# granne/granne

Hardware: AMD Instinct MI355X
Metric: queries/sec (recall@10 alongside), 10M x 100-d angular, batch=1024 (higher is better)
Workload: dtype f32; 1 GPU; C2 (BASELINE.json configs[1]): 10000000 x 100-d f32 angular, i.i.d. uniform components, batch=1024, ef_search=50, k=10; n_elements=10000000, dim=100, batch=1024, ef_search=50, k=10

## Files before the change

granne_amd/_lib.py:

```python
import ctypes as C
import os

from . import build as _build

F32, I8, F16 = 0, 1, 2
UNUSED = 0xFFFFFFFF
BUILD_ALL = 0xFFFFFFFFFFFFFFFF

OK = 0
ERR_INVALID, ERR_HIP, ERR_NO_DEVICE, ERR_OVERFLOW, ERR_IO = -1, -2, -3, -4, -5

OPT_VISITED_SLOTS, OPT_FORCE_SLOW, OPT_SLOW_SLOTS, OPT_SLOW_BLOCKS, OPT_OVERFLOW_SLOTS = 1, 2, 3, 4, 5
OPT_VISITED16, OPT_VISITED16_LG, OPT_LAST_WALKER, OPT_SEARCH_DEPTH, OPT_INLINE_TAILS, OPT_SEEN_MIN = 6, 7, 8, 9, 10, 11
OPT_SKETCH = 12
OPT_COALESCE, OPT_COALESCE_MAX, OPT_COALESCE_WAIT_US, OPT_COALESCED_LAUNCHES, OPT_COALESCED_QUERIES = 13, 14, 15, 16, 17
OPT_LAST_COMPACT_ROWS = 18
OPT_LAST_SPLIT_TAIL = 19
OPT_LAST_SCAN = 20
(SCAN_NONE, SCAN_RING, SCAN_I8, SCAN_I8_CHUNKED, SCAN_B16_7_4, SCAN_B16_13_2, SCAN_B16_16_1, SCAN_B16_CHUNKED, SCAN_F32_52_4,
 SCAN_F32_100_2, SCAN_F32_128_1) = range(11)
EXACT_TOPK_KMAX = 1024
EXACT_TOPK_CAP = 4096
COALESCE_CALL_MAX = 64
COALESCE_MAX = 1024
# ... 42 lines not shown
    "granne_hip_device_count": (i32, [C.POINTER(i32)]),
    "granne_hip_index_create": (i32, [C.POINTER(vp), vp, u64, u32, i32, u32, vp, vp, vp, i32]),
    "granne_hip_index_create_csr": (i32, [C.POINTER(vp), vp, u64, u32, i32, u32, vp, vp, vp, i32]),
    "granne_hip_index_create_device": (i32, [C.POINTER(vp), vp, u64, u32, i32, u32, vp, vp, vp, i32, vp]),
    "granne_hip_index_destroy": (None, [vp]),
    "granne_hip_index_len": (u64, [vp]),
    "granne_hip_index_num_layers": (u32, [vp]),
    "granne_hip_index_layer_len": (u64, [vp, u32]),
    "granne_hip_index_dim": (u32, [vp]),
    "granne_hip_index_dtype": (i32, [vp]),
    "granne_hip_index_device": (i32, [vp]),
    "granne_hip_index_hbm_bytes": (u64, [vp]),
    "granne_hip_index_get_neighbors": (i32, [vp, u64, u32, vp, u32, C.POINTER(u32)]),
    "granne_hip_index_get_element": (i32, [vp, u64, vp]),
    "granne_hip_index_get_sketch": (i32, [vp, u64, u64, vp]),
    "granne_hip_search_batch": (i32, [vp, vp, u32, u32, u32, vp, vp, vp, vp]),
    "granne_hip_search_batch_device": (i32, [vp, vp, u32, u32, u32, vp, vp, vp, vp, vp, vp]),
    "granne_hip_search_batches_device": (i32, [vp, u32, vp, u32, u32, u32, vp, vp, vp, vp, vp, vp]),
    "granne_hip_search_begin_device": (i32, [vp, vp, u32, u32, u32, vp, vp, vp, vp, vp, vp, C.POINTER(u64)]),
    "granne_hip_search_end_device": (i32, [vp, u64, vp]),
    "granne_hip_device_malloc": (i32, [C.POINTER(vp), u64, i32]),
    "granne_hip_device_free": (i32, [vp, i32]),
    "granne_hip_copy_to_device": (i32, [vp, vp, u64, i32, vp]),
    "granne_hip_copy_to_host": (i32, [vp, vp, u64, i32, vp]),
    "granne_hip_stream_create": (i32, [C.POINTER(vp), i32]),
    "granne_hip_stream_destroy": (i32, [vp, i32]),
    "granne_hip_stream_synchronize": (i32, [vp, i32]),
    "granne_hip_event_create": (i32, [vp]),
    "granne_hip_event_destroy": (None, [vp]),
    "granne_hip_event_elapsed_ms": (i32, [vp, vp, vp]),
# ... 134 lines not shown
```

granne_amd/csrc/granne_hip.hip:

```cpp
#include <hip/hip_runtime.h>

#include <atomic>
#include <chrono>
#include <cstdarg>
#include <cstdio>
#include <cstdlib>
#include <cstring>
#include <memory>
#include <mutex>
#include <string>
#include <type_traits>
#include <vector>

#include "../../include/granne_hip.h"
#include "search_kernel.h"
#include "walk_fast.h"
#include "slow_kernel.h"
#include "util_kernels.h"
#include "brute_force.h"
#include "exact_topk.h"
#include "combiner.h"
#include "dev_mem.h"

using namespace granne_hip;
// ... 337 lines not shown
    const uint64_t n = ix->n_elements;
    const size_t bytes = (size_t)n * SKETCH_LINE;
    if (!ix->d_sketch) {
        size_t free_b = 0, total_b = 0;
        if (hipMemGetInfo(&free_b, &total_b) != hipSuccess) {
            (void)hipGetLastError();
            return GRANNE_HIP_OK;
        }
        if ((uint64_t)free_b < (uint64_t)bytes + total_b / 32u) return GRANNE_HIP_OK;
        if (ix->d_sketch.alloc(bytes) != hipSuccess) {
            (void)hipGetLastError();
            return GRANNE_HIP_OK;
        }
        ix->hbm_bytes += bytes;
    }
    hipLaunchKernelGGL(row_sketch_kernel, dim3(grid_for(n, 256)), dim3(256), 0, s, ix->d_elements.as<uint8_t>(), n, ix->row_stride, ix->dim,
                       ix->d_sketch.as<uint8_t>());
    HIP_TRY(hipGetLastError());
    return GRANNE_HIP_OK;
}

static int finish_layers(granne_hip_index* ix, hipStream_t s) {
    std::vector<LayerDev> h(ix->layers.size());
    ix->max_dev_width = 32;
    {
        int r = make_inline_tails(ix, s);
        if (r == 0) r = make_scan_norms(ix, s);
        if (r == 0) r = make_row_sketch(ix, s);
        if (r) return r;
    }
    DevBuf found_buf;
    std::vector<uint32_t> found(h.size(), 0u);
// ... 216 lines not shown
}

extern "C" int granne_hip_index_get_element(const granne_hip_index* ix, uint64_t idx, void* out) {
    if (!ix || !out) return fail(GRANNE_HIP_ERR_INVALID, "null argument");
    if (idx >= ix->n_elements) return fail(GRANNE_HIP_ERR_INVALID, "element index out of range");
    if (ix->se) return se_rows_to_host(*ix->se, idx, 1, 1, (float*)out);
    DeviceGuard g(ix->device);
    HIP_TRY(hipMemcpy(out, ix->d_elements.as<uint8_t>() + idx * ix->row_stride, (size_t)ix->dim * elem_size(ix->dtype),
                      hipMemcpyDeviceToHost));
    return GRANNE_HIP_OK;
}

extern "C" int granne_hip_index_get_sketch(const granne_hip_index* ix, uint64_t first, uint64_t count, void* out) {
    if (!ix || (!out && count)) return fail(GRANNE_HIP_ERR_INVALID, "null argument");
    GRANNE_HIP_COMPACT_UNSUPPORTED(ix, "get_sketch");
    if (!ix->d_sketch) return fail(GRANNE_HIP_ERR_INVALID, "the index holds no row sketches");
    if (first > ix->n_elements || count > ix->n_elements - first) return fail(GRANNE_HIP_ERR_INVALID, "rows out of range");
    if (count == 0) return GRANNE_HIP_OK;
    DeviceGuard g(ix->device);
    HIP_TRY(hipMemcpy(out, ix->d_sketch.as<uint8_t>() + first * SKETCH_LINE, (size_t)count * SKETCH_LINE, hipMemcpyDeviceToHost));
    return GRANNE_HIP_OK;
}

extern "C" int granne_hip_index_set_option(granne_hip_index* ix, int option, uint64_t value) {
    if (!ix) return fail(GRANNE_HIP_ERR_INVALID, "index is null");
    switch (option) {
    case GRANNE_HIP_OPT_VISITED_SLOTS:
        {
            const uint64_t odd = value ? value >> __builtin_ctzll(value) : 1;
            if (value != 0 && (value < 256 || value > 32768 || (odd != 1 && odd != 3)))
// ... 364 lines not shown
    else
        P.S = ef_walk <= 64 ? 1u : ef_walk <= 128 ? 2u : 4u;

    const int vmode = T.opt_visited16 ? (int)T.opt_visited16 : knobs().visited;
    const bool none = vmode == 4 || vmode == 0;
    const bool longest = walk_list_is_long((int)P.S, wide) || wide;
    uint32_t walk_lds;
    if (fast && !trail && ((none && !T.opt_visited_slots) || longest)) {
        const uint32_t touch_max = knobs().touch_max >= 0 ? (uint32_t)knobs().touch_max : 256u;
        const bool touch_shape = P.S == 1 && !wide && !streamed && !(i8 && T.stage_row_bytes != 128);
        P.v16 = (touch_shape && nq <= touch_max) ? 4 : 3;
        const uint64_t seen_min = knobs().seen_min >= 0 ? (uint64_t)knobs().seen_min : T.opt_seen_min;
        if (P.S <= 4 && !wide && !i8 && nq >= seen_min) P.v16 = 5;
        P.cr = P.v16 == 5 && !i8 && sketch_dim_ok(T.dim) && T.d_sketch != nullptr && knobs().compact_rows != 0;
        P.split = P.cr && !wide;
        walk_lds = fast_lds_bytes(i8, streamed, T.dim, T.stage_row_bytes, P.S, 0u, P.v16 == 5, wide);
        const uint32_t least = lds_query_bytes(T.stage_row_bytes) + 64u * 8u;
        if (walk_lds < least) walk_lds = least;
    } else {
        uint32_t want = T.opt_visited_slots ? (uint32_t)T.opt_visited_slots : next_pow2(ef_walk * 64u);
        if (!T.opt_visited_slots) {
            if (want < 1024) want = 1024;
            uint32_t cap = nq >= 4096 ? 4096u : 8192u;
            if (fast && P.S >= 8) cap = 4096u;
            if (want > cap) want = cap;
        }
        P.visited_slots = want;
        P.upper_slots = want < 1024 ? want : 1024;
        if (fast) {
            walk_lds = fast_lds_bytes(i8, streamed, T.dim, T.stage_row_bytes, P.S, P.visited_slots, false, wide);
        } else {
// ... 1282 lines not shown
```

granne_amd/csrc/search_kernel.h:

```cpp
#pragma once

#include "dist.h"
#include "wave_prims.h"
#include "sum_embeddings.h"
#include "f16.h"

namespace granne_hip {

constexpr int DT_F32 = 0;
constexpr int DT_I8 = 1;

struct LayerDev {
    const uint32_t* adj;
    uint64_t len;
    uint32_t width;
    uint32_t flags;
    const uint8_t* adjx;
    uint32_t adjx_stride;
    uint32_t reserved;
};
constexpr uint32_t LAYER_TWIN_ROWS = 1u;

constexpr uint32_t SKETCH_LINE = 128u;
constexpr uint32_t SKETCH_META = 112u;
constexpr uint32_t SKETCH_MAX_DIM = 112u;
__host__ __device__ constexpr bool sketch_dim_ok(uint32_t dim) { return dim == 100u; }

constexpr uint32_t MAX_LAUNCH_BATCHES = 32;
struct BatchIO {
    const uint8_t* queries;
    uint64_t* out_ids;
    float* out_dists;
    uint32_t* out_counts;
    uint64_t* out_stats;
};

struct SearchParams {
    const uint8_t* elements;
    uint64_t n_elements;
    uint32_t dim;
    uint32_t row_bytes;
// ... 548 lines not shown
```

granne_amd/csrc/util_kernels.h:

```cpp
#pragma once

#include "dist.h"
#include "ordered_sum.h"
#include "search_kernel.h"

namespace granne_hip {

__device__ __forceinline__ float sketch_ceil_sqrt(double S) {
    const double T = S * (1.0 + 0x1p-40);
    if (!(T <= (double)3.4028234663852886e38 * (double)3.4028234663852886e38)) return __builtin_inff();
    float f = (float)__builtin_sqrt(T);
    while ((double)f * (double)f < T) f = __uint_as_float(__float_as_uint(f) + 1u);
    while (f > 0.0f) {
        const float g = __uint_as_float(__float_as_uint(f) - 1u);
        if ((double)g * (double)g < T) break;
        f = g;
    }
    return f;
}

__global__ void row_sketch_kernel(const uint8_t* __restrict__ elements, uint64_t n, uint32_t row_stride, uint32_t dim,
                                  uint8_t* __restrict__ out) {
    for (uint64_t row = (uint64_t)blockIdx.x * blockDim.x + threadIdx.x; row < n; row += (uint64_t)gridDim.x * blockDim.x) {
        const float* x = reinterpret_cast<const float*>(elements + row * row_stride);
        uint32_t* o = reinterpret_cast<uint32_t*>(out + row * SKETCH_LINE);
        float m = 0.0f;
        bool finite = true;
        for (uint32_t i = 0; i < dim; ++i) {
            const float a = __builtin_fabsf(x[i]);
            finite = finite && a <= 3.4028234663852886e38f;
            m = a > m ? a : m;
        }
        const float s = finite ? (float)((double)m / 127.0) : 0.0f;
        double se = 0.0, sc = 0.0, sx = 0.0;
        for (uint32_t j = 0; j < SKETCH_META / 4u; ++j) {
            uint32_t w = 0;
            for (uint32_t t = 0; t < 4u; ++t) {
                const uint32_t i = j * 4u + t;
                if (i >= dim) break;
                const double xd = (double)x[i];
                double c = 0.0;
                if (s > 0.0f) {
                    c = __builtin_rint(xd / (double)s);
                    c = c < -127.0 ? -127.0 : (c > 127.0 ? 127.0 : c);
                }
                const double pc = (double)s * c, e = xd - pc;
                se = se + e * e;
                sc = sc + pc * pc;
                sx = sx + xd * xd;
                w |= ((uint32_t)(int32_t)c & 0xFFu) << (8u * t);
            }
            o[j] = w;
        }
        const float inf = __builtin_inff();
        o[SKETCH_META / 4u + 0u] = __float_as_uint(s);
        o[SKETCH_META / 4u + 1u] = __float_as_uint(finite ? sketch_ceil_sqrt(se) : inf);
        o[SKETCH_META / 4u + 2u] = __float_as_uint(finite ? sketch_ceil_sqrt(sc) : inf);
        o[SKETCH_META / 4u + 3u] = __float_as_uint(finite ? sketch_ceil_sqrt(sx) : inf);
    }
}

__global__ void relayout_rows_kernel(const uint8_t* __restrict__ src, uint8_t* __restrict__ dst, uint64_t n,
                                     uint32_t src_bytes, uint32_t dst_bytes) {
    const uint32_t units = dst_bytes >> 4;
    uint64_t total = n * units;
    for (uint64_t t = (uint64_t)blockIdx.x * blockDim.x + threadIdx.x; t < total;
         t += (uint64_t)gridDim.x * blockDim.x) {
        uint64_t row = t / units;
        uint32_t u = (uint32_t)(t - row * units);
        const uint8_t* s = src + row * src_bytes + (uint64_t)u * 16;
        uint32_t avail = (u * 16 < src_bytes) ? min(16u, src_bytes - u * 16) : 0u;
        uint32_t w[4] = {0, 0, 0, 0};
        uint8_t* wb = reinterpret_cast<uint8_t*>(w);
// ... 363 lines not shown
```

granne_amd/csrc/walk_fast.h:

```cpp
#pragma once

#include <type_traits>

#include "slow_kernel.h"

namespace granne_hip {

#ifndef GRANNE_HIP_PHASE_TIMERS
#define GRANNE_HIP_PHASE_TIMERS 0
#endif
#if GRANNE_HIP_PHASE_TIMERS
constexpr uint32_t PHASE_SLOTS = 48, PHASE_QUERIES = 4096;
__device__ uint64_t g_phase[PHASE_QUERIES * PHASE_SLOTS];
#define PT_MARK(i)                                                                   \
    do {                                                                             \
        asm volatile("" ::: "memory");                                               \
        __builtin_amdgcn_sched_barrier(0);                                           \
        const uint64_t now_ = __builtin_amdgcn_s_memtime();                          \
        const uint64_t dt_ = now_ - pt_last;                                         \
        if (pt_bottom) pt_b[i] += dt_; else pt_u[i] += dt_;                          \
        pt_last = now_;                                                              \
        __builtin_amdgcn_sched_barrier(0);                                           \
        asm volatile("" ::: "memory");                                               \
    } while (0)
// ... 182 lines not shown
    uint8_t* lds_q;
    uint64_t* mslot;
    uint32_t* vis_tab;
    uint32_t* vcache;
    float qh[QREG ? NB * 16 : 1];
    float qt[(QREG && TU) ? TU * 4 : 1];
    uint4 qi8[F32 ? 1 : 4 * NBI];
    float sy;
    uint32_t g_nbk, g_ngroups, g_tu;
    static constexpr bool NOVIS = V16 >= 3;
    static constexpr bool TOUCH = V16 == 4;
    static constexpr bool SEEN = V16 == 5;
    static_assert(!WIDE || V16 == 3, "layers of 64 ids: walked without a visited set only");
    static constexpr bool SK = SEEN && XT && sketch_dim_ok((uint32_t)DIM);
    static_assert(CR == 0 || (SK && (CR == 8 || CR == 4) && S <= 4), "the compacted row stage: the sketched launches, 8 or 4 lanes per row");
    int8_t* sk_qc;
    float sk_s, sk_r, sk_n;
    bool sk_on;
    static_assert(V16 == 0 || V16 == 3 || V16 == 4 || V16 == 5, "the exact 32-bit table, or no visited set (4: + rows touched ahead, 5: + revisits skipped before their rows are fetched)");
    typename std::conditional<V16 == 0, VisitedSet, VisitedNone>::type vis;
    List L;
    WalkStats st;
    bool bail;
    uint32_t theta;
#if GRANNE_HIP_PHASE_TIMERS
    uint64_t pt_b[16] = {}, pt_u[16] = {}, pt_last = 0, pt_t0 = 0;
    uint32_t pt_nb = 0, pt_nu = 0, pt_cnt[8] = {0, 0, 0, 0, 0, 0, 0, 0};
    bool pt_bottom = false;
#endif

    __device__ __forceinline__ FastWalker(const SearchParams& p_, uint8_t* smem) : p(p_) {
        lane = threadIdx.x;
        h = lane & 1u;
        R = lane >> 1;
        const uint32_t qb = fast_query_bytes(!F32, GEN, p.dim, p.row_bytes, (uint32_t)S, V16 == 5);
        g_nbk = p.dim / 32u;
        g_ngroups = (g_nbk + GEN_GROUP - 1u) / GEN_GROUP;
        g_tu = ((p.dim & 31u) + 3u) / 4u;
        lds_q = smem;
        mslot = reinterpret_cast<uint64_t*>(smem + qb);
        fimg = reinterpret_cast<uint64_t*>(smem + qb + List::IMAGE_KEYS * 8u);
        vcache = reinterpret_cast<uint32_t*>(smem + qb + List::IMAGE_KEYS * 8u + (LONG_LIST ? FIMG_KEYS * 8u : 0u));
        fkey = KEY_INF;
        nF = nM = 0;
        m_un = 0;
        m_un_key = KEY_INF;
        lost_bits = 0xFFFFFFFFu;
        vis_tab = reinterpret_cast<uint32_t*>(smem + qb + List::IMAGE_KEYS * 8u + (LONG_LIST ? FIMG_KEYS * 8u : 0u) + VSLOTS * 4u);
        st.n_dist = st.n_expand = st.n_adj = 0;
        bail = false;
        sy = 0.0f;
        sk_qc = reinterpret_cast<int8_t*>(vis_tab);
        sk_s = sk_r = sk_n = 0.0f;
        sk_on = false;
        vis.init_walker();
    }

    __device__ __forceinline__ void load_query(uint32_t qi) {
        if constexpr (F32) {
            const float* q = reinterpret_cast<const float*>(query_io(p, qi).q);
            if constexpr (QREG) {
#pragma unroll
                for (int b = 0; b < NB; ++b)
// ... 44 lines not shown
            m = t > m ? t : m;
        }
        const float s = m / 127.0f;
        const float inv = m > 0.0f ? 127.0f / m : 0.0f;
        float c0 = __builtin_rintf(v0 * inv), c1 = __builtin_rintf(v1 * inv);
        c0 = c0 < -127.0f ? -127.0f : (c0 > 127.0f ? 127.0f : c0);
        c1 = c1 < -127.0f ? -127.0f : (c1 > 127.0f ? 127.0f : c1);
        const float e0 = __builtin_fmaf(-s, c0, v0), e1 = __builtin_fmaf(-s, c1, v1);
        float ee = __builtin_fmaf(e1, e1, e0 * e0), nn = __builtin_fmaf(v1, v1, v0 * v0);
        for (int o = 32; o > 0; o >>= 1) {
            ee += __shfl_xor(ee, o, 64);
            nn += __shfl_xor(nn, o, 64);
        }
        sk_qc[lane] = (int8_t)(int)c0;
        sk_qc[lane + 64u] = (int8_t)(int)c1;
        asm volatile("" ::: "memory");
        sk_s = __int_as_float(__builtin_amdgcn_readfirstlane(__float_as_int(s)));
        sk_r = __int_as_float(__builtin_amdgcn_readfirstlane(__float_as_int(__builtin_sqrtf(ee) * (1.0f + 0x1p-8f) + 0x1p-58f)));
        sk_n = __int_as_float(__builtin_amdgcn_readfirstlane(__float_as_int(__builtin_sqrtf(nn) * (1.0f + 0x1p-8f) + 0x1p-58f)));
        sk_on = fin;
    }

    struct RowRegs {
        float4 v[NB ? NB : 1][4];
        float4 vt[GEN ? 8 : (TU ? TU : 1)];
        uint4 x[4 * NBI];
        const uint8_t* row;
    };

    __device__ __forceinline__ void load_group(RowRegs& rr, uint32_t g) {
// ... 47 lines not shown
            const uint8_t* line = p.sketch + (size_t)nb * SKETCH_LINE + h * 64u;
#pragma unroll
            for (int k = 0; k < 4; ++k) rr.v[0][k] = *reinterpret_cast<const float4*>(line + k * 16);
        }
        asm volatile("" ::: "memory");
        int ip = 0;
#pragma unroll
        for (int k = 0; k < 4; ++k) {
            const uint4 qq = *reinterpret_cast<const uint4*>(sk_qc + h * 64u + k * 16);
            ip = dot4_i8(__float_as_uint(rr.v[0][k].x), qq.x, ip);
            ip = dot4_i8(__float_as_uint(rr.v[0][k].y), qq.y, ip);
            ip = dot4_i8(__float_as_uint(rr.v[0][k].z), qq.z, ip);
            ip = dot4_i8(__float_as_uint(rr.v[0][k].w), qq.w, ip);
        }
        ip += pair_swap(ip);
        static_assert(SKETCH_META == 64u + 48u, "s, R, X, N: the last 16 bytes of the odd lane's half");
        const float sx = rr.v[0][3].x, rx = rr.v[0][3].y, xx = rr.v[0][3].z, nx = rr.v[0][3].w;
        const float t = (sk_s * sx) * (float)ip;
        const float nqnx = sk_n * nx;
        const float b = (sk_r * xx + sk_n * rx) + nqnx * 0x1p-17f;
        const float U = t + ((__builtin_fabsf(t) * 0x1p-20f + b * 1.0001f) + 0x1p-20f);
        const float lb = 1.0f - U;
        const uint64_t rm = wave_ballot(go && h != 0u && nqnx < 0x1p100f && lb > __uint_as_float(theta));
        return rm | (rm >> 1);
    }

    __device__ __forceinline__ float finish_rows(RowRegs& rr) {
        float d;
        if constexpr (GEN) {
            float acc[16];
#pragma unroll
            for (int j = 0; j < 16; ++j) acc[j] = 0.0f;
// ... 89 lines not shown
            if (q != q) q = 0.0f;
            const float t = 1.0f - q;
            d = (0.0f <= t) ? t : 0.0f;
        }
        return d;
    }

    static constexpr int CG = CR ? CR : 8;
    static constexpr int CU = 8 / CG;
    static constexpr uint32_t CNG = 64u / CG;
    struct CRows {
        float4 v[NB ? NB : 1][CU];
        float4 vt[TU ? TU : 1];
    };
    __device__ __forceinline__ uint64_t* cr_slots() const { return mslot + CAP; }
    __device__ __forceinline__ void cr_issue(CRows& c, const uint64_t e, const bool act, const uint32_t ct, const uint8_t* xtails) const {
        if (act) {
            const uint8_t* row = p.elements + (size_t)(uint32_t)e * RSTRIDE;
#pragma unroll
            for (int b = 0; b < NB; ++b)
#pragma unroll
                for (int u = 0; u < CU; ++u) c.v[b][u] = *reinterpret_cast<const float4*>(row + b * 128 + (ct * CU + u) * 16u);
            const uint8_t* tp = xtails ? xtails + (uint32_t)(e >> 32) * XTAILB : row + NB * 128;
#pragma unroll
            for (int u = 0; u < TU; ++u) {
                const uint4 t = load_global_u4((gptr_u32)(tp + u * 16));
                c.vt[u] = make_float4(__uint_as_float(t.x), __uint_as_float(t.y), __uint_as_float(t.z), __uint_as_float(t.w));
            }
        }
    }
    __device__ __forceinline__ float cr_finish(const CRows& c, const uint32_t ct) const {
        typedef float f32x2 __attribute__((ext_vector_type(2)));
        f32x2 acc2[2 * CU];
#pragma unroll
        for (int j = 0; j < 2 * CU; ++j) acc2[j] = f32x2{0.0f, 0.0f};
#pragma unroll
        for (int b = 0; b < NB; ++b) {
#pragma unroll
            for (int u = 0; u < CU; ++u) {
                const float4 qq = *reinterpret_cast<const float4*>(lds_q + b * 128 + (ct * CU + u) * 16u);
                acc2[u * 2 + 0] = __builtin_elementwise_fma(f32x2{c.v[b][u].x, c.v[b][u].y}, f32x2{qq.x, qq.y}, acc2[u * 2 + 0]);
                acc2[u * 2 + 1] = __builtin_elementwise_fma(f32x2{c.v[b][u].z, c.v[b][u].w}, f32x2{qq.z, qq.w}, acc2[u * 2 + 1]);
// ... 11 lines not shown
            s = __uint_as_float((uint32_t)__builtin_amdgcn_update_dpp(0, __float_as_int(s), 0x111 , 0xf, 0xf, true) & keep);
#pragma unroll
            for (int j = 0; j < 4 * CU; ++j) s = s + acc[j];
        }
        float r = s;
#pragma unroll
        for (int u = 0; u < TU; ++u) {
            const float4 qq = *reinterpret_cast<const float4*>(lds_q + NB * 128 + u * 16);
            r = __builtin_fmaf(c.vt[u].x, qq.x, r);
            r = __builtin_fmaf(c.vt[u].y, qq.y, r);
            r = __builtin_fmaf(c.vt[u].z, qq.z, r);
            r = __builtin_fmaf(c.vt[u].w, qq.w, r);
        }
        return angular_from_dot(r);
    }
    __device__ __forceinline__ float compact_rows(const uint32_t ns, const uint32_t srank, const bool surv, const uint8_t* xtails) const {
        const uint32_t ct = lane & (uint32_t)(CG - 1), g = lane / (uint32_t)CG;
        const uint64_t* cs = cr_slots();
        float d = 0.0f;
        uint32_t base = 0;
        CRows ra;
#pragma unroll 1
        do {
            const uint32_t sa = base + g;
            const uint64_t ea = cs[sa];
            cr_issue(ra, ea, sa < ns, ct, xtails);
            asm volatile("" ::: "memory");
            const uint32_t rel = srank - base;
            const int from = (int)(((rel & (CNG - 1u)) * (uint32_t)CG + (uint32_t)(CG - 1)) * 4u);
            const float da = cr_finish(ra, ct);
            const float ba = __int_as_float(__builtin_amdgcn_ds_bpermute(from, __float_as_int(da)));
            d = (surv && rel < CNG) ? ba : d;
            base += CNG;
        } while (base < ns);
        return d;
    }

    static constexpr bool LONG = List::LONG;
    static constexpr int LONG_STEPS = CAP >= 4096u ? 7 : 6;
    static constexpr uint32_t FCAP = 63u;
    static constexpr uint32_t FIMG_KEYS = 128u;
// ... 521 lines not shown
            PT_MARK(8);
            PT_COUNT();
            uint64_t ykey = KEY_INF;
            uint32_t ypos = WPOS_NONE, yid = xid;
            for (uint32_t half = 0; half < (WIDE ? 2u : 1u); ++half) {
            if constexpr (WIDE) {
                if (half == 1u) nb = nb_hi;
            }
            const uint64_t unused = wave_ballot(nb == ID_EMPTY);
            const uint32_t nvalid = unused ? ((uint32_t)__builtin_ctzll(unused) >> 1) : 32u;
            st.n_adj += nvalid;
            [[maybe_unused]] uint64_t seenm = 0;
            [[maybe_unused]] uint64_t skipm = 0;
            [[maybe_unused]] uint32_t cr_ns = 0, cr_rank = 0;
            [[maybe_unused]] bool cr_surv = false;
            if constexpr (SEEN) {
                const bool seen = vcache[vcache_slot(nb)] == nb;
                seenm = wave_ballot(seen);
                if constexpr (GEN) {
                    const uint64_t newm = wave_ballot(!seen && nb != ID_EMPTY);
                    const uint32_t fill = newm ? readlane32(nb, (uint32_t)__builtin_ctzll(newm)) : xid;
                    issue_rows((!seen && nb != ID_EMPTY) ? nb : fill, rr);
                } else {
                    bool go = !seen && nb != ID_EMPTY;
                    if constexpr (SK) {
                        if (p.sketch && sk_on && theta < 0x7F800000u) {
                            skipm = sketch_rejects(nb, go, rr);
                            go = go && ((skipm >> lane) & 1ull) == 0ull;
                        }
                    }
                    if constexpr (CR != 0) {
                        const uint64_t sm = wave_ballot(go) & 0xAAAAAAAAAAAAAAAAull;
                        cr_ns = (uint32_t)__popcll(sm);
                        cr_rank = mbcnt64(sm);
                        cr_surv = go && h != 0u;
                        if (cr_surv) cr_slots()[cr_rank] = ((uint64_t)R << 32) | nb;
                    } else if (go) {
                        const uint8_t* tails = nullptr;
                        if constexpr (XT) {
                            if (adjx) tails = adjx + (size_t)xid * Ly.adjx_stride + 128u + R * XTAILB;
                        }
                        issue_rows(nb, rr, tails);
                    }
                }
            } else {
                uint32_t fill = readlane32(nb, 0);
                asm("" : "+v"(fill));
                fill = fill != ID_EMPTY ? fill : xid;
                const uint8_t* tails = nullptr;
                if constexpr (XT) {
                    if (adjx) tails = adjx + (size_t)xid * Ly.adjx_stride + 128u + (nb != ID_EMPTY ? R : 0u) * XTAILB;
// ... 16 lines not shown
                if (nb != ID_EMPTY && !__builtin_amdgcn_inverse_ballot_w64(seenm)) vcache[vcache_slot(nb)] = nb;
            }
            asm volatile("" ::: "memory");
            __builtin_amdgcn_sched_barrier(0);
            PT_MARK(1);

            uint64_t fm;
            if constexpr (SEEN) fm = 0x5555555555555555ull & ~unused & ~seenm;
            else if constexpr (NOVIS) fm = 0x5555555555555555ull & ~unused;
            else fm = wave_ballot(vis.insert(nb, h == 0u && R < nvalid, p.ovf));
            PT_MARK(2);
            PT_WAIT_VM();
            PT_MARK(3);
            float d = 0.0f;
            if constexpr (CR != 0) {
                if (cr_ns) d = compact_rows(cr_ns, cr_rank, cr_surv, adjx ? adjx + (size_t)xid * Ly.adjx_stride + 128u : nullptr);
            } else {
                d = finish_rows(rr);
            }
            if constexpr (TOUCH) {
#pragma unroll
                for (int j = 0; j < NT; ++j) asm volatile("" ::"v"(touched[j]));
                if constexpr (XT) asm volatile("" ::"v"(touched_x));
                const uint32_t tid = next_nb != ID_EMPTY ? next_nb : yid;
                const uint8_t* tb = p.elements + (size_t)tid * RSTRIDE;
                const uint32_t lim = (XT && adjx) ? (uint32_t)NB * 128u : ROWB;
#pragma unroll
                for (int j = 0; j < NT; ++j) {
                    const uint32_t off = h * 128u + (uint32_t)j * 256u;
                    touched[j] = *reinterpret_cast<const uint32_t*>(tb + (off < lim ? off : lim - 4u));
                }
// ... 210 lines not shown
}

template <int DT, int DIM, int S, bool TRAIL = false, int V16 = 0, bool WIDE = false, int CR = 0>
__global__ __launch_bounds__(64, fast_waves_per_simd(DT, DIM, S, WIDE, V16 == 5, CR)) void fast_kernel(const SlowParams P) {
    extern __shared__ __align__(16) uint8_t smem[];
    if constexpr (CR != 0) {
        fast_walk_one<DT, DIM, S, TRAIL, V16, WIDE, CR>(P.sp, blockIdx.x, smem);
    } else if (blockIdx.x < P.sp.nq) {
        fast_walk_one<DT, DIM, S, TRAIL, V16, WIDE, CR>(P.sp, blockIdx.x, smem);
        walker_done(P);
    } else {
        tail_block<DT>(P, smem);
    }
}

__host__ __device__ inline uint32_t fast_lds_bytes(bool i8, bool gen, uint32_t dim, uint32_t row_bytes, uint32_t S, uint32_t visited_slots, bool seen = false, bool wide = false) {
    const bool lng = walk_list_is_long((int)S, wide);
    const uint32_t sk = (seen && !i8 && !gen && !wide && sketch_dim_ok(dim)) ? SKETCH_LINE : 0u;
    return fast_query_bytes(i8, gen, dim, row_bytes, S, seen) + (64u * S + (lng ? 0u : 32u)) * 8u + (lng ? 128u * 8u : 0u) + fast_vcache_slots(seen, sk != 0u, (int)S) * 4u + visited_slots * 4u + sk;
}

}
```

granne_amd/index.py:

```python
import ctypes as C
import os

import numpy as np

from ._lib import ERR_OVERFLOW, EXACT_TOPK_CAP, F16, F32, I8, GranneHipError, check, lib

DEFAULT_MAX_SEARCH = 200
DEFAULT_NUM_ELEMENTS = 10

_ELEMENT_TYPES = {"angular": (F32, np.float32), "angular_int": (I8, np.int8), "angular_f16": (F16, np.float16)}
EMBEDDINGS = "embeddings"


def _p(a):
    return a.ctypes.data_as(C.c_void_p)


def normalize(rows, device=0):
    a = np.array(rows, dtype=np.float32, order="C", copy=True)
    flat = a.reshape(1, -1) if a.ndim == 1 else a
    if flat.size:
        check(lib().granne_hip_normalize_f32(_p(flat), flat.shape[0], flat.shape[1], device))
    return a

# ... 228 lines not shown
    def get_element(self, idx):
        out = np.empty(self.dim, self.np_dtype)
        check(lib().granne_hip_index_get_element(self._h, idx, _p(out)))
        return out

    def hbm_bytes(self):
        return int(lib().granne_hip_index_hbm_bytes(self._h))

    def get_sketch(self, first=0, count=None):
        count = len(self) - first if count is None else count
        out = np.empty((count, 128), np.uint8)
        if lib().granne_hip_index_get_sketch(self._h, first, count, _p(out)) != 0:
            return None
        return out

    def reorder(self):
        order = np.empty(len(self), np.uint64)
        check(lib().granne_hip_index_reorder(self._h, _p(order)))
        return order

    def reorder_by_keys(self, keys):
        k = np.ascontiguousarray(keys, dtype=np.uint64)
        if k.shape != (len(self),):
            raise ValueError("need one key per element")
        order = np.empty(len(self), np.uint64)
        check(lib().granne_hip_index_reorder_by_keys(self._h, _p(k), _p(order)))
        return order

    def set_option(self, option, value):
        check(lib().granne_hip_index_set_option(self._h, option, value))
# ... 219 lines not shown
```

include/granne_hip.h:

```cpp
#ifndef GRANNE_HIP_H
#define GRANNE_HIP_H

#include <stddef.h>
#include <stdint.h>

#ifdef __cplusplus
extern "C" {
#endif

#define GRANNE_HIP_ABI_VERSION 3

enum { GRANNE_HIP_F32 = 0, GRANNE_HIP_I8 = 1, GRANNE_HIP_F16 = 2 };

enum {
    GRANNE_HIP_OK = 0,
    GRANNE_HIP_ERR_INVALID = -1,
    GRANNE_HIP_ERR_HIP = -2,
    GRANNE_HIP_ERR_NO_DEVICE = -3,
    GRANNE_HIP_ERR_OVERFLOW = -4,
    GRANNE_HIP_ERR_IO = -5
};

#define GRANNE_HIP_UNUSED 0xFFFFFFFFu

// ... 19 lines not shown
                                   int device_id, void* stream);

void granne_hip_index_destroy(granne_hip_index* index);

uint64_t granne_hip_index_len(const granne_hip_index* index);
uint32_t granne_hip_index_num_layers(const granne_hip_index* index);
uint64_t granne_hip_index_layer_len(const granne_hip_index* index, uint32_t layer);
uint32_t granne_hip_index_dim(const granne_hip_index* index);
int granne_hip_index_dtype(const granne_hip_index* index);
int granne_hip_index_device(const granne_hip_index* index);
uint64_t granne_hip_index_hbm_bytes(const granne_hip_index* index);
int granne_hip_index_get_neighbors(const granne_hip_index* index, uint64_t node, uint32_t layer,
                                   uint32_t* out_ids, uint32_t cap, uint32_t* out_count);
int granne_hip_index_get_element(const granne_hip_index* index, uint64_t idx, void* out);
int granne_hip_index_get_sketch(const granne_hip_index* index, uint64_t first, uint64_t count, void* out);

int granne_hip_search_batch(const granne_hip_index* index, const void* queries, uint32_t nq,
                            uint32_t max_search, uint32_t num_neighbors, uint64_t* out_ids,
                            float* out_dists, uint32_t* out_counts, uint64_t* out_stats);

int granne_hip_search_batch_device(const granne_hip_index* index, const void* d_queries, uint32_t nq,
                                   uint32_t max_search, uint32_t num_neighbors, uint64_t* d_out_ids,
                                   float* d_out_dists, uint32_t* d_out_counts, uint64_t* d_out_stats,
                                   uint32_t* d_status, void* stream);

int granne_hip_search_batches_device(const granne_hip_index* index, uint32_t n_batches,
                                     const void* const* d_queries, uint32_t nq, uint32_t max_search,
                                     uint32_t num_neighbors, uint64_t* const* d_out_ids,
                                     float* const* d_out_dists, uint32_t* const* d_out_counts,
                                     uint64_t* const* d_out_stats, uint32_t* d_status, void* stream);
// ... 322 lines not shown
```

rust/granne-hip/src/gpu.rs:

```rust
use crate::{angular, angular_int, Index};
use std::marker::PhantomData;
use std::os::raw::{c_char, c_int, c_void};

#[repr(C)] pub struct granne_hip_index { _private: [u8; 0] }
#[repr(C)] pub struct granne_hip_builder { _private: [u8; 0] }
#[repr(C)] pub struct granne_hip_sharded { _private: [u8; 0] }
#[repr(C)] pub struct granne_hip_sum_embeddings { _private: [u8; 0] }
#[repr(C)] pub struct granne_hip_rw_builder { _private: [u8; 0] }

pub const GRANNE_HIP_F32: c_int = 0;
pub const GRANNE_HIP_I8: c_int = 1;
pub const GRANNE_HIP_F16: c_int = 2;
pub const GRANNE_HIP_BUILD_ALL: u64 = u64::MAX;

#[repr(C)]
pub struct granne_hip_build_config {
    pub layer_multiplier: f32,
    pub expected_num_elements: u64,
    pub num_neighbors: u32,
    pub max_search: u32,
    pub reinsert_elements: c_int,
    pub show_progress: c_int,
    pub batch_max: u32,
    pub batch_div: u32,
// ... 12 lines not shown
        elements_bytes: *const c_void, elements_len: u64, dtype: c_int, device_id: c_int) -> c_int;
    fn granne_hip_index_load_files(out: *mut *mut granne_hip_index, index_path: *const c_char,
        elements_path: *const c_char, dtype: c_int, device_id: c_int) -> c_int;
    fn granne_hip_index_save(index: *const granne_hip_index, index_path: *const c_char, elements_path: *const c_char) -> c_int;
    fn granne_hip_index_encode(index: *const granne_hip_index, out_bytes: *mut *mut c_void, out_len: *mut u64) -> c_int;
    fn granne_hip_bytes_free(bytes: *mut c_void);
    fn granne_hip_index_destroy(index: *mut granne_hip_index);
    fn granne_hip_index_len(index: *const granne_hip_index) -> u64;
    fn granne_hip_index_num_layers(index: *const granne_hip_index) -> u32;
    fn granne_hip_index_layer_len(index: *const granne_hip_index, layer: u32) -> u64;
    fn granne_hip_index_dim(index: *const granne_hip_index) -> u32;
    fn granne_hip_index_get_neighbors(index: *const granne_hip_index, node: u64, layer: u32,
        out_ids: *mut u32, cap: u32, out_count: *mut u32) -> c_int;
    fn granne_hip_index_get_element(index: *const granne_hip_index, idx: u64, out: *mut c_void) -> c_int;
    fn granne_hip_index_get_sketch(index: *const granne_hip_index, first: u64, count: u64, out: *mut c_void) -> c_int;
    fn granne_hip_search(index: *const granne_hip_index, query: *const c_void, max_search: u32,
        num_neighbors: u32, out_ids: *mut u64, out_dists: *mut f32, out_count: *mut u32) -> c_int;
    fn granne_hip_search_batch(index: *const granne_hip_index, queries: *const c_void, nq: u32,
        max_search: u32, num_neighbors: u32, out_ids: *mut u64, out_dists: *mut f32,
        out_counts: *mut u32, out_stats: *mut u64) -> c_int;
    fn granne_hip_refine_device(refine_index: *const granne_hip_index, d_queries: *const c_void, nq: u32,
        d_cand_ids: *const u64, d_cand_counts: *const u32, m: u32, k: u32, d_out_ids: *mut u64,
        d_out_dists: *mut f32, d_out_counts: *mut u32, d_refine_status: *mut u32, stream: *mut c_void) -> c_int;
    fn granne_hip_search_refined_batch_device(walk_index: *const granne_hip_index,
        refine_index: *const granne_hip_index, d_walk_queries: *const c_void, d_refine_queries: *const c_void,
        nq: u32, max_search: u32, refine_from: u32, k: u32, d_out_ids: *mut u64, d_out_dists: *mut f32,
        d_out_counts: *mut u32, d_out_stats: *mut u64, d_status: *mut u32, d_refine_status: *mut u32,
        stream: *mut c_void) -> c_int;
    fn granne_hip_search_refined_batch(walk_index: *const granne_hip_index, refine_index: *const granne_hip_index,
        walk_queries: *const c_void, refine_queries: *const c_void, nq: u32, max_search: u32, refine_from: u32,
// ... 763 lines not shown
```

Baseline: 16.08 million queries/s.

## Store each row's 16-byte tail in its sketch line to skip tail loads

Changes the per-row sketch layout so the line keeps s, R and X in the third unit and copies the row's last four floats into the final 16 bytes; the norm bound N is now derived from X+R rather than stored. During the walk, rows that pass the sketch filter stage their tail in LDS from the already-loaded sketch line. The compacted-row distance pass then reads the tail from LDS instead of issuing a separate global tail load per surviving row. This costs 512 bytes of extra LDS per block and a slightly looser norm bound, and get_sketch now recomputes the old layout on the fly while a new get_walk_sketch exposes the stored one.

```diff
diff --git a/granne_amd/_lib.py b/granne_amd/_lib.py
--- a/granne_amd/_lib.py
+++ b/granne_amd/_lib.py
@@ -80,6 +80,7 @@
     "granne_hip_index_get_neighbors": (i32, [vp, u64, u32, vp, u32, C.POINTER(u32)]),
     "granne_hip_index_get_element": (i32, [vp, u64, vp]),
     "granne_hip_index_get_sketch": (i32, [vp, u64, u64, vp]),
+    "granne_hip_index_get_walk_sketch": (i32, [vp, u64, u64, vp]),
     "granne_hip_search_batch": (i32, [vp, vp, u32, u32, u32, vp, vp, vp, vp]),
     "granne_hip_search_batch_device": (i32, [vp, vp, u32, u32, u32, vp, vp, vp, vp, vp, vp]),
     "granne_hip_search_batches_device": (i32, [vp, u32, vp, u32, u32, u32, vp, vp, vp, vp, vp, vp]),
diff --git a/granne_amd/csrc/granne_hip.hip b/granne_amd/csrc/granne_hip.hip
--- a/granne_amd/csrc/granne_hip.hip
+++ b/granne_amd/csrc/granne_hip.hip
@@ -375,8 +375,8 @@
         }
         ix->hbm_bytes += bytes;
     }
-    hipLaunchKernelGGL(row_sketch_kernel, dim3(grid_for(n, 256)), dim3(256), 0, s, ix->d_elements.as<uint8_t>(), n, ix->row_stride, ix->dim,
-                       ix->d_sketch.as<uint8_t>());
+    hipLaunchKernelGGL(row_sketch_kernel<true>, dim3(grid_for(n, 256)), dim3(256), 0, s, ix->d_elements.as<uint8_t>(), (uint64_t)0, n,
+                       ix->row_stride, ix->dim, ix->d_sketch.as<uint8_t>());
     HIP_TRY(hipGetLastError());
     return GRANNE_HIP_OK;
 }
@@ -623,6 +623,26 @@
 extern "C" int granne_hip_index_get_sketch(const granne_hip_index* ix, uint64_t first, uint64_t count, void* out) {
     if (!ix || (!out && count)) return fail(GRANNE_HIP_ERR_INVALID, "null argument");
     GRANNE_HIP_COMPACT_UNSUPPORTED(ix, "get_sketch");
+    if (!ix->d_sketch) return fail(GRANNE_HIP_ERR_INVALID, "the index holds no row sketches");
+    if (first > ix->n_elements || count > ix->n_elements - first) return fail(GRANNE_HIP_ERR_INVALID, "rows out of range");
+    if (count == 0) return GRANNE_HIP_OK;
+    DeviceGuard g(ix->device);
+    const uint64_t step = count < (1ull << 20) ? count : (1ull << 20);
+    DevBuf tmp;
+    HIP_TRY(tmp.alloc((size_t)step * SKETCH_LINE));
+    for (uint64_t done = 0; done < count; done += step) {
+        const uint64_t m = count - done < step ? count - done : step;
+        hipLaunchKernelGGL(row_sketch_kernel<false>, dim3(grid_for(m, 256)), dim3(256), 0, 0, ix->d_elements.as<uint8_t>(), first + done, m,
+                           ix->row_stride, ix->dim, tmp.as<uint8_t>());
+        HIP_TRY(hipGetLastError());
+        HIP_TRY(hipMemcpy((uint8_t*)out + (size_t)done * SKETCH_LINE, tmp.as<uint8_t>(), (size_t)m * SKETCH_LINE, hipMemcpyDeviceToHost));
+    }
+    return GRANNE_HIP_OK;
+}
+
+extern "C" int granne_hip_index_get_walk_sketch(const granne_hip_index* ix, uint64_t first, uint64_t count, void* out) {
+    if (!ix || (!out && count)) return fail(GRANNE_HIP_ERR_INVALID, "null argument");
+    GRANNE_HIP_COMPACT_UNSUPPORTED(ix, "get_walk_sketch");
     if (!ix->d_sketch) return fail(GRANNE_HIP_ERR_INVALID, "the index holds no row sketches");
     if (first > ix->n_elements || count > ix->n_elements - first) return fail(GRANNE_HIP_ERR_INVALID, "rows out of range");
     if (count == 0) return GRANNE_HIP_OK;
@@ -1017,7 +1037,7 @@
         if (P.S <= 4 && !wide && !i8 && nq >= seen_min) P.v16 = 5;
         P.cr = P.v16 == 5 && !i8 && sketch_dim_ok(T.dim) && T.d_sketch != nullptr && knobs().compact_rows != 0;
         P.split = P.cr && !wide;
-        walk_lds = fast_lds_bytes(i8, streamed, T.dim, T.stage_row_bytes, P.S, 0u, P.v16 == 5, wide);
+        walk_lds = fast_lds_bytes(i8, streamed, T.dim, T.stage_row_bytes, P.S, 0u, P.v16 == 5, wide, P.cr && !wide);
         const uint32_t least = lds_query_bytes(T.stage_row_bytes) + 64u * 8u;
         if (walk_lds < least) walk_lds = least;
     } else {
diff --git a/granne_amd/csrc/search_kernel.h b/granne_amd/csrc/search_kernel.h
--- a/granne_amd/csrc/search_kernel.h
+++ b/granne_amd/csrc/search_kernel.h
@@ -24,7 +24,13 @@
 constexpr uint32_t SKETCH_LINE = 128u;
 constexpr uint32_t SKETCH_META = 112u;
 constexpr uint32_t SKETCH_MAX_DIM = 112u;
+constexpr uint32_t SKETCH_WALK_META = 100u;
+constexpr uint32_t SKETCH_WALK_TAIL = 112u;
+constexpr uint32_t SKETCH_WALK_TAIL_BYTES = 16u;
 __host__ __device__ constexpr bool sketch_dim_ok(uint32_t dim) { return dim == 100u; }
+static_assert(SKETCH_WALK_TAIL == 64u + 3u * 16u && SKETCH_WALK_TAIL + SKETCH_WALK_TAIL_BYTES == SKETCH_LINE, "the tail: the odd lane's fourth unit");
+static_assert(SKETCH_WALK_META == 64u + 2u * 16u + 4u && SKETCH_WALK_META + 12u == SKETCH_WALK_TAIL, "s, R, X: words 1..3 of the odd lane's third unit");
+static_assert(sketch_dim_ok(SKETCH_WALK_META) && (SKETCH_WALK_META % 32u) * 4u == SKETCH_WALK_TAIL_BYTES, "100 codes, and a tail of 100 % 32 floats");
 
 constexpr uint32_t MAX_LAUNCH_BATCHES = 32;
 struct BatchIO {
diff --git a/granne_amd/csrc/util_kernels.h b/granne_amd/csrc/util_kernels.h
--- a/granne_amd/csrc/util_kernels.h
+++ b/granne_amd/csrc/util_kernels.h
@@ -19,10 +19,11 @@
     return f;
 }
 
-__global__ void row_sketch_kernel(const uint8_t* __restrict__ elements, uint64_t n, uint32_t row_stride, uint32_t dim,
+template <bool WALK>
+__global__ void row_sketch_kernel(const uint8_t* __restrict__ elements, uint64_t first, uint64_t n, uint32_t row_stride, uint32_t dim,
                                   uint8_t* __restrict__ out) {
     for (uint64_t row = (uint64_t)blockIdx.x * blockDim.x + threadIdx.x; row < n; row += (uint64_t)gridDim.x * blockDim.x) {
-        const float* x = reinterpret_cast<const float*>(elements + row * row_stride);
+        const float* x = reinterpret_cast<const float*>(elements + (first + row) * row_stride);
         uint32_t* o = reinterpret_cast<uint32_t*>(out + row * SKETCH_LINE);
         float m = 0.0f;
         bool finite = true;
@@ -53,10 +54,16 @@
             o[j] = w;
         }
         const float inf = __builtin_inff();
-        o[SKETCH_META / 4u + 0u] = __float_as_uint(s);
-        o[SKETCH_META / 4u + 1u] = __float_as_uint(finite ? sketch_ceil_sqrt(se) : inf);
-        o[SKETCH_META / 4u + 2u] = __float_as_uint(finite ? sketch_ceil_sqrt(sc) : inf);
-        o[SKETCH_META / 4u + 3u] = __float_as_uint(finite ? sketch_ceil_sqrt(sx) : inf);
+        constexpr uint32_t META = (WALK ? SKETCH_WALK_META : SKETCH_META) / 4u;
+        o[META + 0u] = __float_as_uint(s);
+        o[META + 1u] = __float_as_uint(finite ? sketch_ceil_sqrt(se) : inf);
+        o[META + 2u] = __float_as_uint(finite ? sketch_ceil_sqrt(sc) : inf);
+        if constexpr (WALK) {
+            const uint32_t* xb = reinterpret_cast<const uint32_t*>(x) + (dim - SKETCH_WALK_TAIL_BYTES / 4u);
+            for (uint32_t t = 0; t < SKETCH_WALK_TAIL_BYTES / 4u; ++t) o[SKETCH_WALK_TAIL / 4u + t] = xb[t];
+        } else {
+            o[META + 3u] = __float_as_uint(finite ? sketch_ceil_sqrt(sx) : inf);
+        }
     }
 }
 
diff --git a/granne_amd/csrc/walk_fast.h b/granne_amd/csrc/walk_fast.h
--- a/granne_amd/csrc/walk_fast.h
+++ b/granne_amd/csrc/walk_fast.h
@@ -220,6 +220,8 @@
     static_assert(!WIDE || V16 == 3, "layers of 64 ids: walked without a visited set only");
     static constexpr bool SK = SEEN && XT && sketch_dim_ok((uint32_t)DIM);
     static_assert(CR == 0 || (SK && (CR == 8 || CR == 4) && S <= 4), "the compacted row stage: the sketched launches, 8 or 4 lanes per row");
+    static_assert(!SK || (XTAILB == SKETCH_WALK_TAIL_BYTES && TU == 1), "a sketch line carries its row's whole tail: one 16-byte unit");
+    static constexpr uint32_t CR_TAILS_BYTES = CR ? 32u * XTAILB : 0u;
     int8_t* sk_qc;
     float sk_s, sk_r, sk_n;
     bool sk_on;
@@ -246,13 +248,13 @@
         lds_q = smem;
         mslot = reinterpret_cast<uint64_t*>(smem + qb);
         fimg = reinterpret_cast<uint64_t*>(smem + qb + List::IMAGE_KEYS * 8u);
-        vcache = reinterpret_cast<uint32_t*>(smem + qb + List::IMAGE_KEYS * 8u + (LONG_LIST ? FIMG_KEYS * 8u : 0u));
+        vcache = reinterpret_cast<uint32_t*>(smem + qb + List::IMAGE_KEYS * 8u + (LONG_LIST ? FIMG_KEYS * 8u : 0u) + CR_TAILS_BYTES);
         fkey = KEY_INF;
         nF = nM = 0;
         m_un = 0;
         m_un_key = KEY_INF;
         lost_bits = 0xFFFFFFFFu;
-        vis_tab = reinterpret_cast<uint32_t*>(smem + qb + List::IMAGE_KEYS * 8u + (LONG_LIST ? FIMG_KEYS * 8u : 0u) + VSLOTS * 4u);
+        vis_tab = reinterpret_cast<uint32_t*>(smem + qb + List::IMAGE_KEYS * 8u + (LONG_LIST ? FIMG_KEYS * 8u : 0u) + CR_TAILS_BYTES + VSLOTS * 4u);
         st.n_dist = st.n_expand = st.n_adj = 0;
         bail = false;
         sy = 0.0f;
@@ -327,6 +329,7 @@
         }
         sk_qc[lane] = (int8_t)(int)c0;
         sk_qc[lane + 64u] = (int8_t)(int)c1;
+        static_assert(DIM <= (int)SKETCH_WALK_META, "the query's codes end where a line's s, R, X begin");
         asm volatile("" ::: "memory");
         sk_s = __int_as_float(__builtin_amdgcn_readfirstlane(__float_as_int(s)));
         sk_r = __int_as_float(__builtin_amdgcn_readfirstlane(__float_as_int(__builtin_sqrtf(ee) * (1.0f + 0x1p-8f) + 0x1p-58f)));
@@ -404,8 +407,10 @@
             ip = dot4_i8(__float_as_uint(rr.v[0][k].w), qq.w, ip);
         }
         ip += pair_swap(ip);
-        static_assert(SKETCH_META == 64u + 48u, "s, R, X, N: the last 16 bytes of the odd lane's half");
-        const float sx = rr.v[0][3].x, rx = rr.v[0][3].y, xx = rr.v[0][3].z, nx = rr.v[0][3].w;
+        static_assert(SKETCH_WALK_META == 64u + 32u + 4u && SKETCH_WALK_TAIL == 64u + 48u, "s, R, X and the tail in the odd lane's half");
+        const float sx = rr.v[0][2].y, rx = rr.v[0][2].z, xx = rr.v[0][2].w;
+        const uint32_t nxb = __float_as_uint(xx + rx) + 1u;
+        const float nx = __uint_as_float(nxb < 0x7F800000u ? nxb : 0x7F800000u);
         const float t = (sk_s * sx) * (float)ip;
         const float nqnx = sk_n * nx;
         const float b = (sk_r * xx + sk_n * rx) + nqnx * 0x1p-17f;
@@ -525,18 +530,22 @@
         float4 vt[TU ? TU : 1];
     };
     __device__ __forceinline__ uint64_t* cr_slots() const { return mslot + CAP; }
-    __device__ __forceinline__ void cr_issue(CRows& c, const uint64_t e, const bool act, const uint32_t ct, const uint8_t* xtails) const {
+    __device__ __forceinline__ float4* cr_tails() const { return reinterpret_cast<float4*>(mslot + List::IMAGE_KEYS); }
+    __device__ __forceinline__ void cr_issue(CRows& c, const uint64_t e, const bool act, const uint32_t ct, const uint8_t* xtails,
+                                             const bool gtail = true) const {
         if (act) {
             const uint8_t* row = p.elements + (size_t)(uint32_t)e * RSTRIDE;
 #pragma unroll
             for (int b = 0; b < NB; ++b)
 #pragma unroll
                 for (int u = 0; u < CU; ++u) c.v[b][u] = *reinterpret_cast<const float4*>(row + b * 128 + (ct * CU + u) * 16u);
-            const uint8_t* tp = xtails ? xtails + (uint32_t)(e >> 32) * XTAILB : row + NB * 128;
-#pragma unroll
-            for (int u = 0; u < TU; ++u) {
-                const uint4 t = load_global_u4((gptr_u32)(tp + u * 16));
-                c.vt[u] = make_float4(__uint_as_float(t.x), __uint_as_float(t.y), __uint_as_float(t.z), __uint_as_float(t.w));
+            if (gtail) {
+                const uint8_t* tp = xtails ? xtails + (uint32_t)(e >> 32) * XTAILB : row + NB * 128;
+#pragma unroll
+                for (int u = 0; u < TU; ++u) {
+                    const uint4 t = load_global_u4((gptr_u32)(tp + u * 16));
+                    c.vt[u] = make_float4(__uint_as_float(t.x), __uint_as_float(t.y), __uint_as_float(t.z), __uint_as_float(t.w));
+                }
             }
         }
     }
@@ -578,9 +587,11 @@
         }
         return angular_from_dot(r);
     }
-    __device__ __forceinline__ float compact_rows(const uint32_t ns, const uint32_t srank, const bool surv, const uint8_t* xtails) const {
+    __device__ __forceinline__ float compact_rows(const uint32_t ns, const uint32_t srank, const bool surv, const uint8_t* xtails,
+                                                  const bool sketched) const {
         const uint32_t ct = lane & (uint32_t)(CG - 1), g = lane / (uint32_t)CG;
         const uint64_t* cs = cr_slots();
+        const float4* const lt = cr_tails();
         float d = 0.0f;
         uint32_t base = 0;
         CRows ra;
@@ -588,7 +599,11 @@
         do {
             const uint32_t sa = base + g;
             const uint64_t ea = cs[sa];
-            cr_issue(ra, ea, sa < ns, ct, xtails);
+            if (sketched) {
+#pragma unroll
+                for (int u = 0; u < TU; ++u) ra.vt[u] = lt[sa * (uint32_t)TU + (uint32_t)u];
+            }
+            cr_issue(ra, ea, sa < ns, ct, xtails, !sketched);
             asm volatile("" ::: "memory");
             const uint32_t rel = srank - base;
             const int from = (int)(((rel & (CNG - 1u)) * (uint32_t)CG + (uint32_t)(CG - 1)) * 4u);
@@ -1140,6 +1155,7 @@
             [[maybe_unused]] uint64_t skipm = 0;
             [[maybe_unused]] uint32_t cr_ns = 0, cr_rank = 0;
             [[maybe_unused]] bool cr_surv = false;
+            [[maybe_unused]] bool cr_sketched = false;
             if constexpr (SEEN) {
                 const bool seen = vcache[vcache_slot(nb)] == nb;
                 seenm = wave_ballot(seen);
@@ -1153,6 +1169,7 @@
                         if (p.sketch && sk_on && theta < 0x7F800000u) {
                             skipm = sketch_rejects(nb, go, rr);
                             go = go && ((skipm >> lane) & 1ull) == 0ull;
+                            cr_sketched = true;
                         }
                     }
                     if constexpr (CR != 0) {
@@ -1160,7 +1177,10 @@
                         cr_ns = (uint32_t)__popcll(sm);
                         cr_rank = mbcnt64(sm);
                         cr_surv = go && h != 0u;
-                        if (cr_surv) cr_slots()[cr_rank] = ((uint64_t)R << 32) | nb;
+                        if (cr_surv) {
+                            cr_slots()[cr_rank] = ((uint64_t)R << 32) | nb;
+                            if (cr_sketched) cr_tails()[cr_rank] = rr.v[0][3];
+                        }
                     } else if (go) {
                         const uint8_t* tails = nullptr;
                         if constexpr (XT) {
@@ -1207,7 +1227,7 @@
             PT_MARK(3);
             float d = 0.0f;
             if constexpr (CR != 0) {
-                if (cr_ns) d = compact_rows(cr_ns, cr_rank, cr_surv, adjx ? adjx + (size_t)xid * Ly.adjx_stride + 128u : nullptr);
+                if (cr_ns) d = compact_rows(cr_ns, cr_rank, cr_surv, adjx ? adjx + (size_t)xid * Ly.adjx_stride + 128u : nullptr, cr_sketched);
             } else {
                 d = finish_rows(rr);
             }
@@ -1448,10 +1468,10 @@
     }
 }
 
-__host__ __device__ inline uint32_t fast_lds_bytes(bool i8, bool gen, uint32_t dim, uint32_t row_bytes, uint32_t S, uint32_t visited_slots, bool seen = false, bool wide = false) {
+__host__ __device__ inline uint32_t fast_lds_bytes(bool i8, bool gen, uint32_t dim, uint32_t row_bytes, uint32_t S, uint32_t visited_slots, bool seen = false, bool wide = false, bool cr = false) {
     const bool lng = walk_list_is_long((int)S, wide);
     const uint32_t sk = (seen && !i8 && !gen && !wide && sketch_dim_ok(dim)) ? SKETCH_LINE : 0u;
-    return fast_query_bytes(i8, gen, dim, row_bytes, S, seen) + (64u * S + (lng ? 0u : 32u)) * 8u + (lng ? 128u * 8u : 0u) + fast_vcache_slots(seen, sk != 0u, (int)S) * 4u + visited_slots * 4u + sk;
+    return fast_query_bytes(i8, gen, dim, row_bytes, S, seen) + (64u * S + (lng ? 0u : 32u)) * 8u + (lng ? 128u * 8u : 0u) + fast_vcache_slots(seen, sk != 0u, (int)S) * 4u + visited_slots * 4u + sk + (cr ? 32u * SKETCH_WALK_TAIL_BYTES : 0u);
 }
 
 }
diff --git a/granne_amd/index.py b/granne_amd/index.py
--- a/granne_amd/index.py
+++ b/granne_amd/index.py
@@ -266,6 +266,13 @@
             return None
         return out
 
+    def get_walk_sketch(self, first=0, count=None):
+        count = len(self) - first if count is None else count
+        out = np.empty((count, 128), np.uint8)
+        if lib().granne_hip_index_get_walk_sketch(self._h, first, count, _p(out)) != 0:
+            return None
+        return out
+
     def reorder(self):
         order = np.empty(len(self), np.uint64)
         check(lib().granne_hip_index_reorder(self._h, _p(order)))
diff --git a/include/granne_hip.h b/include/granne_hip.h
--- a/include/granne_hip.h
+++ b/include/granne_hip.h
@@ -57,6 +57,7 @@
                                    uint32_t* out_ids, uint32_t cap, uint32_t* out_count);
 int granne_hip_index_get_element(const granne_hip_index* index, uint64_t idx, void* out);
 int granne_hip_index_get_sketch(const granne_hip_index* index, uint64_t first, uint64_t count, void* out);
+int granne_hip_index_get_walk_sketch(const granne_hip_index* index, uint64_t first, uint64_t count, void* out);
 
 int granne_hip_search_batch(const granne_hip_index* index, const void* queries, uint32_t nq,
                             uint32_t max_search, uint32_t num_neighbors, uint64_t* out_ids,
diff --git a/rust/granne-hip/src/gpu.rs b/rust/granne-hip/src/gpu.rs
--- a/rust/granne-hip/src/gpu.rs
+++ b/rust/granne-hip/src/gpu.rs
@@ -50,6 +50,7 @@
         out_ids: *mut u32, cap: u32, out_count: *mut u32) -> c_int;
     fn granne_hip_index_get_element(index: *const granne_hip_index, idx: u64, out: *mut c_void) -> c_int;
     fn granne_hip_index_get_sketch(index: *const granne_hip_index, first: u64, count: u64, out: *mut c_void) -> c_int;
+    fn granne_hip_index_get_walk_sketch(index: *const granne_hip_index, first: u64, count: u64, out: *mut c_void) -> c_int;
     fn granne_hip_search(index: *const granne_hip_index, query: *const c_void, max_search: u32,
         num_neighbors: u32, out_ids: *mut u64, out_dists: *mut f32, out_count: *mut u32) -> c_int;
     fn granne_hip_search_batch(index: *const granne_hip_index, queries: *const c_void, nq: u32,
```

Result: faster. 16.41 million queries/s (median of 6 runs) (+2.1%).
